# zhangyi-3/UCDIR

Hardware: AMD Instinct MI355X
Metric: restored images/sec at 50-step p_sample_loop, 256x256 SID (higher is better)
Workload: dtype bf16

## Files before the change

ucdir_amd/csrc/engine.hip:

```cpp
#include <hip/hip_runtime.h>

#include <cmath>
#include <cstdio>
#include <cstring>
#include <map>
#include <mutex>
#include <set>
#include <array>
#include <atomic>
#include <memory>
#include <string>
#include <vector>

#include "../../include/ucdir_hip.h"
#include "cgemm.hip.h"
#include "conv_halo.hip.h"
#include "akgm_halo.hip.h"
#include "akgm_pre.hip.h"
#include "akgm_ws.hip.h"
#include "akgm_ws32.hip.h"
#include "akgm_ws64.hip.h"
#include "conv_ws.hip.h"
#include "conv_sk.hip.h"
#include "conv_ws128.hip.h"
#include "flash_attn2.hip.h"
#include "qkv_ws.hip.h"
#include "common.h"
#include "misc.hip.h"
#include "fewstep.hip.h"
#include "image_metrics.hip.h"
#include "pack.h"

static thread_local std::string g_err;
static int fail(const std::string& m) { g_err = m; return 1; }
#define HIPC(x)                                                                                   \
    do {                                                                                          \
        hipError_t e_ = (x);                                                                      \
        if (e_ != hipSuccess) {                                                                   \
            throw std::runtime_error(std::string(#x) + ": " + hipGetErrorString(e_));             \
        }                                                                                         \
    } while (0)
#define API_BEGIN try {
#define API_END                                                                                   \
    }                                                                                             \
    catch (const std::exception& e) { return fail(e.what()); }                                    \
    catch (...) { return fail("unknown error"); }                                                 \
    return 0;

static void require(bool c, const std::string& m) { if (!c) throw std::runtime_error(m); }

struct DevGuard {
    int prev = -1; bool changed = false;
    explicit DevGuard(int dev) {
        HIPC(hipGetDevice(&prev));
        if (prev != dev) { HIPC(hipSetDevice(dev)); changed = true; }
    }
    ~DevGuard() { if (changed) (void)hipSetDevice(prev); }
};

struct DevPool {
    std::vector<void*> ptrs;
    int64_t bytes = 0;
    void* alloc(size_t n, bool zero = true) {
        void* p = nullptr;
        if (n == 0) n = 16;
        HIPC(hipMalloc(&p, n));
        if (zero) HIPC(hipMemset(p, 0, n));
        ptrs.push_back(p); bytes += (int64_t)n;
        return p;
    }
    template <typename T> T* upload(const std::vector<T>& v) {
        T* p = (T*)alloc(v.size() * sizeof(T), false);
        if (!v.empty()) HIPC(hipMemcpy(p, v.data(), v.size() * sizeof(T), hipMemcpyHostToDevice));
        return p;
    }
    static constexpr size_t STAT_CAP = 1 << 21;
    stat_t* stat_slab = nullptr; size_t stat_used = 0;
    stat_t* alloc_stats(int B) {
        if (!stat_slab) stat_slab = (stat_t*)alloc(STAT_CAP * sizeof(stat_t), true);
        const size_t n = (size_t)2 * UCDIR_STAT_SLOTS * B;
        if (stat_used + n > STAT_CAP) throw std::runtime_error("DevPool: statistics slab exhausted");
        stat_t* p = stat_slab + stat_used; stat_used += n;
        return p;
    }
    void zero_stats(hipStream_t st) { if (stat_used) HIPC(hipMemsetAsync(stat_slab, 0, stat_used * sizeof(stat_t), st)); }
    void release() { for (void* p : ptrs) (void)hipFree(p); ptrs.clear(); bytes = 0; stat_slab = nullptr; stat_used = 0; }
    ~DevPool() { release(); }
};

struct ConvW {
    bf16_t* A = nullptr; float* bias = nullptr; float* Tb = nullptr; float* Tg = nullptr;
    int rows_pad = 0, Kpad = 0, ntaps = 0, cin = 0, cout = 0, TM = 128; bool fold = false;
    bf16_t* Aup = nullptr; int Kup = 0;
    bf16_t* A10 = nullptr; float* bias_res = nullptr;
    bf16_t* Aws = nullptr;
    bf16_t* Aws128 = nullptr;
    bf16_t* Aqkv = nullptr;
    bf16_t* Atile = nullptr;
    bf16_t* Ask[2] = {nullptr, nullptr}; bf16_t* Ask_up[2] = {nullptr, nullptr};
    long long sk_up_stride[2] = {0, 0};
    bf16_t* Ask1x1 = nullptr;
};
struct AkgmW {
    bf16_t* A = nullptr; float* bias = nullptr; float* Tb = nullptr; float* Tg = nullptr;
    float* Tbb = nullptr;
    bf16_t* Apre = nullptr;
    bf16_t* Aws32 = nullptr;
    bf16_t* Aws64 = nullptr;
    int C = 0, cg = 0, Kpad = 0;
};

static int pick_tm(int cout) { return cout >= 128 ? 128 : 64; }

static ConvW upload_conv(DevPool& pool, const float* w, const float* bias, const float* gamma, const float* beta,
                         int cout, int cin, int ks) {
    ConvW W;
    W.TM = pick_tm(cout);
    PackedConv P = pack_conv(w, bias, gamma, beta, cout, cin, ks, W.TM);
    W.A = pool.upload(P.A); W.bias = pool.upload(P.bias);
    W.fold = gamma != nullptr;
    if (W.fold) { W.Tb = pool.upload(P.Tb); W.Tg = pool.upload(P.Tg); }
    W.rows_pad = P.rows_pad; W.Kpad = P.Kpad; W.ntaps = P.ntaps; W.cin = cin; W.cout = cout;
    if (ks == 3 && cin == 64 && cout == 64 && P.Kpad == 576) W.Aws = pool.upload(pack_conv_ws(P));
    if (ks == 3 && cin % 32 == 0 && P.Kpad == 9 * cin && P.rows_pad % W.TM == 0) W.Atile = pool.upload(pack_conv_tiled(P, W.TM));
    if (ks == 3 && cin % 32 == 0 && P.Kpad == 9 * cin && cout % 128 == 0) {
        W.Ask[0] = pool.upload(pack_conv_sk(P.A, 1, P.rows_pad, P.Kpad, cin, 9, 1));
        if (cout % 256 == 0) W.Ask[1] = pool.upload(pack_conv_sk(P.A, 1, P.rows_pad, P.Kpad, cin, 9, 2));
    }
    if (ks == 1 && cin % 32 == 0 && P.Kpad == cin && cout % 128 == 0 && gamma == nullptr) W.Ask1x1 = pool.upload(pack_conv_sk(P.A, 1, P.rows_pad, P.Kpad, cin, 1, 1));
    if (ks == 1 && cout == 3 * cin && gamma != nullptr && (cin == 256 || cin == 512) && P.Kpad == cin && P.rows_pad >= cout) W.Aqkv = pool.upload(pack_qkv_ws(P, cin));
    return W;
}
static void upload_upconv(DevPool& pool, ConvW& W, const float* w, const float* bias) {
    PackedConv P = pack_upconv(w, bias, W.cout, W.cin, W.TM);
    W.Aup = pool.upload(P.A); W.Kup = P.Kpad;
    for (int mw = 1; mw <= 2; ++mw)
        if (W.cin % 32 == 0 && W.cout % (128 * mw) == 0) {
            std::vector<bf16_t> img = pack_conv_sk(P.A, 4, P.rows_pad, P.Kpad, W.cin, 4, mw);
            W.sk_up_stride[mw - 1] = (long long)((img.size() - (size_t)4 * 4 * mw * 2 * 512) / 4);
            W.Ask_up[mw - 1] = pool.upload(img);
        }
}
static AkgmW upload_akgm(DevPool& pool, const float* wsp, const float* bsp, const float* gamma, const float* beta, int C) {
    PackedAkgm P = pack_akgm(wsp, bsp, gamma, beta, C, 0);
    AkgmW W;
    W.A = pool.upload(P.A); W.bias = pool.upload(P.bias); W.Tb = pool.upload(P.Tb); W.Tg = pool.upload(P.Tg);
    W.C = C; W.cg = P.cg; W.Kpad = P.Kpad;
    {
        std::vector<float> tbb(P.Tb.size());
// ... 11 lines not shown
struct Profiler {
    bool on = false;
    std::vector<ProfEntry> entries;
    std::vector<hipEvent_t> pool; size_t used = 0;
    hipEvent_t get() {
        if (used == pool.size()) { hipEvent_t e; HIPC(hipEventCreate(&e)); pool.push_back(e); }
        return pool[used++];
    }
    ~Profiler() { for (auto e : pool) (void)hipEventDestroy(e); }
};
static Profiler g_prof;

template <int TM, int EPI, int MODE>
static void launch_one(const GemmP& p, dim3 grid, size_t lds, hipStream_t st) {
    hipLaunchKernelGGL((cgemm_kernel<TM, EPI, MODE>), grid, dim3(CG_THREADS), lds, st, p);
}

template <typename K> static void set_lds_attr(K* k, int bytes, bool abs0 = false) {
    HIPC(hipFuncSetAttribute((const void*)k, hipFuncAttributeMaxDynamicSharedMemorySize, bytes));
    if (abs0) {
        hipFuncAttributes fa;
        HIPC(hipFuncGetAttributes(&fa, (const void*)k));
        require(fa.sharedSizeBytes == 0, "a kernel with absolute LDS addressing has static __shared__ memory: its dynamic smem[] no longer starts at offset 0");
    }
}
template <int TM> static void set_cgemm_attrs() {
    set_lds_attr(cgemm_kernel<TM, EPI_STD, MODE_S1>, 100 * 1024, true); set_lds_attr(cgemm_kernel<TM, EPI_STD, MODE_DOWN>, 100 * 1024, true);
    set_lds_attr(cgemm_kernel<TM, EPI_STD, MODE_UP>, 100 * 1024, true); set_lds_attr(cgemm_kernel<TM, EPI_STD, MODE_PLAIN>, 100 * 1024, true);
    set_lds_attr(cgemm_kernel<TM, EPI_STD, MODE_S1C>, 100 * 1024, true); set_lds_attr(cgemm_kernel<TM, EPI_AKGM, MODE_S1>, 100 * 1024, true);
}
#define SPLITK_MAX_WGS 512
#define SK_MAX_GRID 256
#define SCRATCH_BYTES ((size_t)2 * SK_MAX_GRID * 65536 * sizeof(float))
static std::map<int, float*> g_splitk_buf;
static std::mutex g_static_mu;
static void ensure_kernel_attrs() {
    std::lock_guard<std::mutex> lk(g_static_mu);
    static std::set<int> done;
    int dev = 0;
    HIPC(hipGetDevice(&dev));
    if (done.count(dev)) return;
    set_cgemm_attrs<64>(); set_cgemm_attrs<128>();
    set_lds_attr(conv3x3_halo_kernel<128, false>, hc_lds_bytes<128>());
    set_lds_attr(conv3x3_halo_kernel<64, false>, hc_lds_bytes<64>());
    set_lds_attr(conv3x3_halo_kernel<64, true>, hc_lds_bytes<64>());
    set_lds_attr(akgm_halo_stage_kernel, AH_LDS); set_lds_attr(akgm_halo_kernel<true>, AH_LDS);
    set_lds_attr(akgm_pre_kernel<8>, AkPre<8>::LDS);
    set_lds_attr(akgm_ws_kernel<8>, AkWs::LDS); set_lds_attr(akgm_ws_kernel<16>, AkWs::LDS);
    set_lds_attr(akgm_ws32_kernel<32>, AkWs32::LDS); set_lds_attr(akgm_ws32_kernel<16>, AkWs32::LDS); set_lds_attr(akgm_ws32_kernel<8>, AkWs32::LDS);
    set_lds_attr(akgm_ws64_kernel<2, 8, true>, 160 * 1024); set_lds_attr(akgm_ws64_kernel<4, 8, true>, 160 * 1024);
    set_lds_attr(qkv_ws_kernel<256>, QkvWs::LDS); set_lds_attr(qkv_ws_kernel<512>, QkvWs::LDS);
    set_lds_attr(conv_ws_kernel, CvWs::LDS);
    set_lds_attr(conv_ws128_kernel, CvWs128::LDS);
    set_lds_attr(conv_sk_kernel<2, 8, 9>, 160 * 1024); set_lds_attr(conv_sk_kernel<2, 8, 4>, 160 * 1024);
    set_lds_attr(conv_sk_kernel<1, 8, 9>, 160 * 1024); set_lds_attr(conv_sk_kernel<1, 8, 4>, 160 * 1024);
    set_lds_attr(conv_sk_kernel<1, 4, 9>, 80 * 1024, true); set_lds_attr(conv_sk_kernel<1, 4, 4>, 80 * 1024, true);

    set_lds_attr(final_conv_kernel, 160 * 1024);
    set_lds_attr(flash_attn2_kernel<1, false>, fa_lds_bytes(128), true); set_lds_attr(flash_attn2_kernel<1, true>, fa_lds_bytes(128), true);
    set_lds_attr(flash_attn2_kernel<2, false>, fa_lds_bytes(256), true); set_lds_attr(flash_attn2_kernel<2, true>, fa_lds_bytes(256), true);
    set_lds_attr(flash_attn2_kernel<3, false>, fa_lds_bytes(384), true); set_lds_attr(flash_attn2_kernel<3, true>, fa_lds_bytes(384), true);
    set_lds_attr(flash_attn2_kernel<4, false>, fa_lds_bytes(512), true); set_lds_attr(flash_attn2_kernel<4, true>, fa_lds_bytes(512), true);
    done.insert(dev);
}

static void gemm_work(const GemmP& p, int epi, double& flops, double& bytes) {
    const double cols = ((p.cols_mode == COLS_PLAIN) ? (double)p.W : (double)p.H * p.W) * (p.up_phase ? 4.0 : 1.0);
    if (epi == EPI_AKGM) {
        const double C = 8.0 * p.cg;
        flops = 2.0 * 9 * C * C * cols * p.nbatch;
        bytes = (2.0 * C * cols * 2 + C * cols * 2 + cols * 32) * p.nbatch + 9.0 * C * C * 2;
    } else {
        const double K = (double)p.ntaps * p.cg;
        flops = 2.0 * K * p.nfeat * cols * p.nbatch;
        double in_cols = cols;
        if (p.cols_mode == COLS_DOWN) in_cols = cols * 4; else if (p.cols_mode == COLS_UP) in_cols = cols / 4;
        bytes = ((double)p.cg * in_cols * 2 + (double)p.nfeat * cols * (p.out_f32 ? 4 : 2) + (p.res ? (double)p.nfeat * cols * 2 : 0)) * p.nbatch
                + (p.a_bstride ? (double)p.nfeat * K * 2 * p.nbatch : (double)p.nfeat * K * 2);
    }
}

static void launch_cgemm_impl(const GemmP& p, int TM, int epi, hipStream_t st);
static void launch_cgemm(const GemmP& p, int TM, int epi, hipStream_t st) {
    if (!g_prof.on) { launch_cgemm_impl(p, TM, epi, st); return; }
    ProfEntry e;
    int mode = p.cols_mode; if (mode == COLS_S1 && p.in_compact) mode = MODE_S1C;
    e.key = (TM == 128 ? 100 : 0) + (epi == EPI_AKGM ? 10 : 0) + (epi == EPI_AKGM ? 0 : mode);
    gemm_work(p, epi, e.flops, e.bytes);
    e.dH = p.H; e.dW = p.W; e.dCin = p.cg * p.ntaps; e.dCout = p.nfeat;
    e.e0 = g_prof.get(); e.e1 = g_prof.get();
    HIPC(hipEventRecord(e.e0, st));
    launch_cgemm_impl(p, TM, epi, st);
    HIPC(hipEventRecord(e.e1, st));
    g_prof.entries.push_back(e);
}

static void launch_cgemm_impl(const GemmP& p0, int TM, int epi, hipStream_t st) {
    GemmP p = p0;
#ifdef UCDIR_TIMING
    static unsigned long long* cgdbg = nullptr;
    if (!cgdbg) HIPC(hipMalloc((void**)&cgdbg, 64 * 8));
    HIPC(hipMemsetAsync(cgdbg, 0, 64 * 8, st));
    p.dbg = cgdbg;
    struct Pr { unsigned long long* d; hipStream_t s; int mode, TM, nk; ~Pr() {
        unsigned long long h[64]; (void)hipStreamSynchronize(s); (void)hipMemcpy(h, d, sizeof(h), hipMemcpyDeviceToHost);
        const int n = (int)h[63]; fprintf(stderr, "CGEMM TIMING mode=%d TM=%d nk=%d n=%d:", mode, TM, nk, n);
// ... 364 lines not shown
    if (!dbgbuf) HIPC(hipMalloc((void**)&dbgbuf, 256 * 8));
    HIPC(hipMemset(dbgbuf, 0, 256 * 8));
    p.dbg = dbgbuf;
#endif
    int tm_run = w.TM;
    if (halo && tm_run == 128 && p.nbatch * p.tiles * p.rowtiles < 256) {
        tm_run = 64; p.rowtiles = w.rows_pad / 64;
    }
    static const bool fuse_res = !getenv("UCDIR_NO_FUSED_RES");
    bool did_res = false;
    if (halo && !upph && tm_run == 64 && w.TM == 64 && w.A10 && res_out && fuse_res) {
        p.A = w.A10; p.a_ld = 10 * cin; p.res_fused = 1; p.bias2 = w.bias_res;
        p.out2 = res_out->p; p.out2_bstride = res_out->bstride(); p.out2_ld = res_out->C;
        did_res = true;
    }
    const bool dual = did_res;
    static const bool use_atile = !getenv("UCDIR_NO_ATILE");
    if (use_atile && halo && !upph && !did_res && tm_run == w.TM && w.Atile && w.ntaps == 9) p.A_tiled = w.Atile;
    static const bool use_cws128 = !getenv("UCDIR_NO_CONV_WS128");
    if (use_cws128 && did_res && w.Aws128 && cin == 128 && x0.C == 64 && x1 && x1->C == 64 && !res && !p.out_nchw && y.H % 8 == 0 && y.W % 16 == 0 &&
        y.C == 64 && (g_persist_grid > 0 || (long long)y.B * (y.H / 8) * (y.W / 16) >= 4LL * num_cus())) {
        p.A = w.Aws128; p.alt_A = w.Aws128 + (size_t)2 * 72 * 2 * 32 * 8;
        p.th = 8; p.tw = 16; p.tiles_x = y.W / 16; p.tiles_y = y.H / 8;
        const int ntiles = y.B * p.tiles_x * p.tiles_y, ncu = num_cus();
        const int grid = ntiles < ncu ? ntiles : ncu;
#ifdef UCDIR_TIMING
        {
            static unsigned long long* dbgbuf = nullptr;
            if (!dbgbuf) HIPC(hipMalloc((void**)&dbgbuf, 256 * 8));
            HIPC(hipMemset(dbgbuf, 0, 256 * 8));
            p.dbg = dbgbuf;
            hipLaunchKernelGGL(conv_ws128_kernel, dim3(grid), dim3(CvWs128::THREADS), CvWs128::LDS, st, p);
            unsigned long long h[256];
            HIPC(hipStreamSynchronize(st));
            HIPC(hipMemcpy(h, dbgbuf, sizeof(h), hipMemcpyDeviceToHost));
            const int n = (int)h[255];
            fprintf(stderr, "CONV_WS128 TIMING n=%d:", n);
            for (int i = 1; i < n && i < 255; ++i) fprintf(stderr, " %llu", h[i] - h[i - 1]);
            fprintf(stderr, "\n");
            return did_res;
        }
#endif
        if (g_prof.on) {
            ProfEntry e; e.key = 24; gemm_work(p, EPI_STD, e.flops, e.bytes);
            { const double cols = (double)p.H * p.W * p.nbatch; e.flops += 2.0 * p.cg * p.nfeat * cols; e.bytes += 2.0 * p.cg * p.nfeat + 2.0 * p.nfeat * cols; }
            e.dH = p.H; e.dW = p.W; e.dCin = p.cg; e.dCout = p.nfeat;
            e.e0 = g_prof.get(); e.e1 = g_prof.get();
            HIPC(hipEventRecord(e.e0, st));
            hipLaunchKernelGGL(conv_ws128_kernel, dim3(grid), dim3(CvWs128::THREADS), CvWs128::LDS, st, p);
            HIPC(hipEventRecord(e.e1, st));
            g_prof.entries.push_back(e);
        } else {
            hipLaunchKernelGGL(conv_ws128_kernel, dim3(grid), dim3(CvWs128::THREADS), CvWs128::LDS, st, p);
        }
        HIPC(hipGetLastError());
        return did_res;
    }
    if (halo && !did_res && !p.out_nchw && w.cout % 8 == 0) {
        const int taps = upph ? 4 : 9, tps = 256 / tm_run;
        const int ks = choose_ksplit(p.nbatch * p.tiles * p.rowtiles, cin / HC_BK, (taps + tps - 1) / tps,
                                     (double)y.B * y.H * y.W * w.cout);
        if (ks > 1) { p.ksplit = ks; p.partial = splitk_scratch(); }
    }
    static const bool tail_res = !getenv("UCDIR_NO_TAIL_RES");
    if (halo && !upph && !did_res && res_out && wres && tail_res && !p.out_nchw && wres->ntaps == 1 &&
        wres->rows_pad >= p.rowtiles * tm_run) {
        p.alt_blocks = p.nbatch * p.tiles * p.rowtiles;
        p.alt_A = wres->A; p.alt_a_ld = wres->Kpad; p.bias2 = wres->bias;
        p.out2 = res_out->p; p.out2_bstride = res_out->bstride(); p.out2_ld = res_out->C;
        did_res = true;
    }
    static const bool use_cws = !getenv("UCDIR_NO_CONV_WS");
    if (use_cws && halo && !upph && !did_res && !dual && w.Aws && !x1 && !res && !p.out_nchw && p.ksplit <= 1 && !p.alt_blocks &&
        y.H % 16 == 0 && y.W % 16 == 0 && x0.C == 64 && y.C == 64 &&
        (g_persist_grid > 0 || (long long)y.B * (y.H / 16) * (y.W / 16) >= 4LL * num_cus())) {
        p.A = w.Aws; p.th = 16; p.tw = 16; p.tiles_x = y.W / 16; p.tiles_y = y.H / 16;
        const int ntiles = y.B * p.tiles_x * p.tiles_y, ncu = num_cus();
        const int grid = ntiles < ncu ? ntiles : ncu;
#ifdef UCDIR_TIMING
        {
            static unsigned long long* dbgbuf = nullptr;
            if (!dbgbuf) HIPC(hipMalloc((void**)&dbgbuf, 512 * 8));
            HIPC(hipMemset(dbgbuf, 0, 512 * 8));
            p.dbg = dbgbuf;
            hipLaunchKernelGGL(conv_ws_kernel, dim3(grid), dim3(HC_THREADS), CvWs::LDS, st, p);
            unsigned long long h[512];
            HIPC(hipStreamSynchronize(st));
            HIPC(hipMemcpy(h, dbgbuf, sizeof(h), hipMemcpyDeviceToHost));
            for (int w = 0; w < 2; ++w) {
                const int n = (int)h[w * 256 + 255];
                fprintf(stderr, "CONV_WS TIMING %s n=%d:", w ? "late" : "early", n);
                for (int i = 1; i < n && i < 255; ++i) fprintf(stderr, " %llu", h[w * 256 + i] - h[w * 256 + i - 1]);
                fprintf(stderr, "\n");
            }
            return did_res;
        }
#endif
        if (g_prof.on) {
            ProfEntry e; e.key = 23; gemm_work(p, EPI_STD, e.flops, e.bytes);
            e.dH = p.H; e.dW = p.W; e.dCin = p.cg; e.dCout = p.nfeat;
            e.e0 = g_prof.get(); e.e1 = g_prof.get();
            HIPC(hipEventRecord(e.e0, st));
            hipLaunchKernelGGL(conv_ws_kernel, dim3(grid), dim3(HC_THREADS), CvWs::LDS, st, p);
            HIPC(hipEventRecord(e.e1, st));
            g_prof.entries.push_back(e);
        } else {
// ... 479 lines not shown
}

static const std::vector<float>& W_(ucdir_ctx* c, const std::string& name, size_t expect) {
    auto it = c->host.find(name);
    require(it != c->host.end(), "missing weight: " + name);
    require(it->second.v.size() == expect, "weight " + name + " has wrong size");
    return it->second.v;
}

static void finalize_weights(ucdir_ctx* c) {
    const auto& cfg = c->cfg;
    const int inner = cfg.inner_channel;
    c->wpool.release();
    c->lw.assign(c->layers.size(), LayerW());
    c->mlp_w1 = c->wpool.upload(W_(c, "noise_level_mlp.1.weight", (size_t)4 * inner * inner));
    c->mlp_b1 = c->wpool.upload(W_(c, "noise_level_mlp.1.bias", (size_t)4 * inner));
    c->mlp_w2 = c->wpool.upload(W_(c, "noise_level_mlp.3.weight", (size_t)4 * inner * inner));
    c->mlp_b2 = c->wpool.upload(W_(c, "noise_level_mlp.3.bias", (size_t)inner));
    std::vector<float> tw;
    int nb = 0;
    for (size_t li = 0; li < c->layers.size(); ++li) {
        const LayerDesc& d = c->layers[li];
        LayerW& w = c->lw[li];
        if (d.kind == "stem") {
            const auto& sw = W_(c, d.name + ".weight", (size_t)d.cout * d.cin * 9);
            require(d.cin == 6, "stem expects in_channel == 6 (cat[cond, x_t])");
            std::vector<float> t((size_t)54 * d.cout);
            for (int o = 0; o < d.cout; ++o) for (int ci = 0; ci < 6; ++ci) for (int k = 0; k < 9; ++k)
                t[(size_t)(k * 6 + ci) * d.cout + o] = sw[((size_t)o * 6 + ci) * 9 + k];
            require(d.cout % 64 == 0, "stem: inner_channel must be a multiple of 64");
            w.stem_w = c->wpool.upload(pack_stem_frags(t, W_(c, d.name + ".bias", (size_t)d.cout), 6, d.cout));
        } else if (d.kind == "down" || d.kind == "up") {
            w.conv = upload_conv(c->wpool, W_(c, d.name + ".conv.weight", (size_t)d.cout * d.cin * 9).data(),
                                 W_(c, d.name + ".conv.bias", d.cout).data(), nullptr, nullptr, d.cout, d.cin, 3);
            if (d.kind == "up") upload_upconv(c->wpool, w.conv, W_(c, d.name + ".conv.weight", (size_t)d.cout * d.cin * 9).data(),
                                              W_(c, d.name + ".conv.bias", d.cout).data());
        } else {
            const std::string r = d.name + ".res_block.";
            w.block_index = nb++;
            w.conv = upload_conv(c->wpool, W_(c, r + "conv1.weight", (size_t)d.cout * d.cin * 9).data(),
                                 W_(c, r + "conv1.bias", d.cout).data(), W_(c, r + "norm1.weight", d.cin).data(),
                                 W_(c, r + "norm1.bias", d.cin).data(), d.cout, d.cin, 3);
            w.has_res = d.cin != d.cout;
            if (w.has_res) {
                w.resconv = upload_conv(c->wpool, W_(c, r + "res_conv.weight", (size_t)d.cout * d.cin).data(),
                                        W_(c, r + "res_conv.bias", d.cout).data(), nullptr, nullptr, d.cout, d.cin, 1);
                if (w.conv.TM == 64 && d.cin % 64 == 0 && w.conv.Kpad == 9 * d.cin) {
                    PackedConv P = pack_conv(W_(c, r + "conv1.weight", (size_t)d.cout * d.cin * 9).data(), nullptr,
                                             W_(c, r + "norm1.weight", d.cin).data(), W_(c, r + "norm1.bias", d.cin).data(),
                                             d.cout, d.cin, 3, 64);
                    const std::vector<bf16_t> a10 = pack_conv_res10(P, W_(c, r + "res_conv.weight", (size_t)d.cout * d.cin).data());
                    w.conv.A10 = c->wpool.upload(a10);
                    if (d.cin == 128 && d.cout == 64) w.conv.Aws128 = c->wpool.upload(pack_conv_ws128(a10));
                    w.conv.bias_res = w.resconv.bias;
                }
            }
            w.sp = upload_akgm(c->wpool, W_(c, r + "spdyconv.weight", (size_t)8 * d.cout * (d.cout / 8) * 9).data(),
                               W_(c, r + "spdyconv.bias", (size_t)8 * d.cout).data(), W_(c, r + "norm2.weight", d.cout).data(),
                               W_(c, r + "norm2.bias", d.cout).data(), d.cout);
            std::vector<float> gw;
            for (const char* s : {"conv2.0.weight", "conv2.0.bias", "conv2.2.weight", "conv2.2.bias"}) {
                const auto& v = c->host.at(r + s).v;
                gw.insert(gw.end(), v.begin(), v.end());
            }
            require(gw.size() == 48 + 16 + 576 + 8, "guide branch weights have wrong size");
            w.gw = c->wpool.upload(gw);
            for (const char* s : {"noise_func.0.weight", "noise_func.0.bias", "noise_func.2.weight", "noise_func.2.bias"}) {
                const auto& v = c->host.at(r + s).v;
                tw.insert(tw.end(), v.begin(), v.end());
            }
            if (d.attn) {
                const std::string a = d.name + ".attn.";
                const std::vector<float> wf = fold_out_into_v(W_(c, a + "qkv.weight", (size_t)3 * d.cout * d.cout).data(),
                                                              W_(c, a + "out.weight", (size_t)d.cout * d.cout).data(), d.cout);
                w.qkv = upload_conv(c->wpool, wf.data(), nullptr,
                                    W_(c, a + "norm.weight", d.cout).data(), W_(c, a + "norm.bias", d.cout).data(),
                                    3 * d.cout, d.cout, 1);
                w.outp = upload_conv(c->wpool, W_(c, a + "out.weight", (size_t)d.cout * d.cout).data(),
                                     W_(c, a + "out.bias", d.cout).data(), nullptr, nullptr, d.cout, d.cout, 1);
            }
        }
    }
    c->nblocks = nb;
    require(tw.size() == (size_t)nb * (8 * inner + 8 + 64 + 8), "time weights have wrong size");
    c->tw = c->wpool.upload(tw);
    const int fc = inner * cfg.channel_mults[0];
    c->fin_gamma = c->wpool.upload(W_(c, "final_conv.0.weight", fc));
    c->fin_beta = c->wpool.upload(W_(c, "final_conv.0.bias", fc));
    c->fin_conv = upload_conv(c->wpool, W_(c, "final_conv.3.weight", (size_t)cfg.out_channel * fc * 9).data(),
                              W_(c, "final_conv.3.bias", cfg.out_channel).data(), nullptr, nullptr, cfg.out_channel, fc, 3);
    if (cfg.out_channel <= 4 && fc % 32 == 0) {
        c->fin_w = c->wpool.upload(pack_final_frags(W_(c, "final_conv.3.weight", (size_t)cfg.out_channel * fc * 9).data(), cfg.out_channel, fc));
        c->fin_b = c->wpool.upload(W_(c, "final_conv.3.bias", cfg.out_channel));
    }
    c->host.clear();
    c->finalized = true;
}

static int level_dim(int d, int level) { return d >> level; }

struct ActPlanner {
    DevPool& pool; int B; bool reuse;
    std::map<std::array<int, 3>, std::vector<bf16_t*>> free_;
    Act get(int h, int w, int C, bool stats = true) {
        Act a; a.B = B; a.H = h; a.W = w; a.C = C;
        auto& fl = free_[{h, w, C}];
// ... 581 lines not shown
}

int32_t ucdir_op_conv(const float* x0, int32_t c0, const float* x1, int32_t c1, int32_t B, int32_t H, int32_t W,
                      const float* w_host, const float* bias_host, const float* gamma_host, const float* beta_host,
                      int32_t cout, int32_t ksize, int32_t mode, int32_t silu, const float* residual, float* y,
                      double* stats_out_host, void* stream) {
    API_BEGIN
    ensure_kernel_attrs();
    hipStream_t st = (hipStream_t)stream;
    DevPool pool;
    Act a0 = act_from_nchw(pool, x0, B, c0, H, W, st, true);
    Act a1; if (x1) a1 = act_from_nchw(pool, x1, B, c1, H, W, st, true);
    int Ho = H, Wo = W;
    if (mode == COLS_DOWN) { Ho = H / 2; Wo = W / 2; } else if (mode == COLS_UP) { Ho = 2 * H; Wo = 2 * W; }
    Act out = make_act(pool, B, Ho, Wo, cout);
    Act res; if (residual) res = act_from_nchw(pool, residual, B, cout, Ho, Wo, st, false);
    ConvW w = upload_conv(pool, w_host, bias_host, gamma_host, beta_host, cout, c0 + (x1 ? c1 : 0), ksize);
    if (mode == COLS_UP && ksize == 3) upload_upconv(pool, w, w_host, bias_host);
    run_conv(w, a0, x1 ? &a1 : nullptr, out, mode, silu, residual ? &res : nullptr, true, st);
    hipLaunchKernelGGL(act_to_nchw_kernel, dim3(2048), dim3(256), 0, st, out.p, y, B, cout, Ho, Wo);
    HIPC(hipGetLastError());
    std::vector<stat_t> sfx;
    if (stats_out_host) { sfx.resize((size_t)2 * UCDIR_STAT_SLOTS * B); HIPC(hipMemcpyAsync(sfx.data(), out.stats, sizeof(stat_t) * sfx.size(), hipMemcpyDeviceToHost, st)); }
    HIPC(hipStreamSynchronize(st));
    if (stats_out_host)
        for (int bb = 0; bb < B; ++bb)
            for (int q = 0; q < 2; ++q) {
                stat_t acc = 0;
                for (int k = 0; k < UCDIR_STAT_SLOTS; ++k) acc += sfx[((size_t)bb * UCDIR_STAT_SLOTS + k) * 2 + q];
                stats_out_host[bb * 2 + q] = (double)acc / UCDIR_STAT_SCALE;
            }
    API_END
}

int32_t ucdir_op_conv_res(const float* x0, int32_t c0, const float* x1, int32_t c1, int32_t B, int32_t H, int32_t W,
                          const float* w_host, const float* bias_host, const float* gamma_host, const float* beta_host,
                          const float* wres_host, const float* bres_host, int32_t cout, int32_t silu,
                          float* y, float* yres, double* stats_out_host, void* stream) {
    API_BEGIN
    ensure_kernel_attrs();
    hipStream_t st = (hipStream_t)stream;
    DevPool pool;
    const int cin = c0 + (x1 ? c1 : 0);
    Act a0 = act_from_nchw(pool, x0, B, c0, H, W, st, true);
    Act a1; if (x1) a1 = act_from_nchw(pool, x1, B, c1, H, W, st, true);
    Act out = make_act(pool, B, H, W, cout), rout = make_act(pool, B, H, W, cout, false);
    ConvW w = upload_conv(pool, w_host, bias_host, gamma_host, beta_host, cout, cin, 3);
    ConvW wr = upload_conv(pool, wres_host, bres_host, nullptr, nullptr, cout, cin, 1);
    if (w.TM == 64 && cin % 64 == 0 && w.Kpad == 9 * cin) {
        PackedConv P = pack_conv(w_host, nullptr, gamma_host, beta_host, cout, cin, 3, 64);
        const std::vector<bf16_t> a10 = pack_conv_res10(P, wres_host);
        w.A10 = pool.upload(a10); w.bias_res = wr.bias;
        if (cin == 128 && cout == 64) w.Aws128 = pool.upload(pack_conv_ws128(a10));
    }
    const bool did = run_conv(w, a0, x1 ? &a1 : nullptr, out, COLS_S1, silu, nullptr, true, st, nullptr, 0, 0, &rout, &wr);
    if (!did) run_conv(wr, a0, x1 ? &a1 : nullptr, rout, COLS_S1, 0, nullptr, false, st);
    hipLaunchKernelGGL(act_to_nchw_kernel, dim3(2048), dim3(256), 0, st, out.p, y, B, cout, H, W);
    hipLaunchKernelGGL(act_to_nchw_kernel, dim3(2048), dim3(256), 0, st, rout.p, yres, B, cout, H, W);
    HIPC(hipGetLastError());
    std::vector<stat_t> sfx;
    if (stats_out_host) { sfx.resize((size_t)2 * UCDIR_STAT_SLOTS * B); HIPC(hipMemcpyAsync(sfx.data(), out.stats, sizeof(stat_t) * sfx.size(), hipMemcpyDeviceToHost, st)); }
    HIPC(hipStreamSynchronize(st));
    if (stats_out_host)
        for (int bb = 0; bb < B; ++bb)
            for (int q = 0; q < 2; ++q) {
                stat_t acc = 0;
                for (int k = 0; k < UCDIR_STAT_SLOTS; ++k) acc += sfx[((size_t)bb * UCDIR_STAT_SLOTS + k) * 2 + q];
                stats_out_host[bb * 2 + q] = (double)acc / UCDIR_STAT_SCALE;
            }
    API_END
}

int32_t ucdir_op_akgm(const float* h, const float* att, const float* res, int32_t B, int32_t C, int32_t H, int32_t W,
                      const float* wsp_host, const float* bsp_host, const float* gamma_host, const float* beta_host,
                      float* y, double* stats_out_host, void* stream) {
    API_BEGIN
    ensure_kernel_attrs();
    hipStream_t st = (hipStream_t)stream;
    DevPool pool;
    Act ah = act_from_nchw(pool, h, B, C, H, W, st, true);
    Act ar = act_from_nchw(pool, res, B, C, H, W, st, false);
    Act out = make_act(pool, B, H, W, C);
    float* G = (float*)pool.alloc((size_t)B * H * W * 8 * 4);
    hipLaunchKernelGGL(nchw8_to_compact_kernel, dim3(1024), dim3(256), 0, st, att, G, B, H, W);
    std::vector<float> ones((size_t)B * 8, 1.f);
    float* attw = pool.upload(ones);
    AkgmW w = upload_akgm(pool, wsp_host, bsp_host, gamma_host, beta_host, C);
    float* tcbuf = (float*)pool.alloc((size_t)B * (9 * 8 * C + 2) * sizeof(float), false);
    run_akgm(w, ah, G, attw, ar, out, tcbuf, st);
    hipLaunchKernelGGL(act_to_nchw_kernel, dim3(2048), dim3(256), 0, st, out.p, y, B, C, H, W);
    HIPC(hipGetLastError());
    std::vector<stat_t> sfx;
    if (stats_out_host) { sfx.resize((size_t)2 * UCDIR_STAT_SLOTS * B); HIPC(hipMemcpyAsync(sfx.data(), out.stats, sizeof(stat_t) * sfx.size(), hipMemcpyDeviceToHost, st)); }
    HIPC(hipStreamSynchronize(st));
    if (stats_out_host)
        for (int bb = 0; bb < B; ++bb)
            for (int q = 0; q < 2; ++q) {
                stat_t acc = 0;
                for (int k = 0; k < UCDIR_STAT_SLOTS; ++k) acc += sfx[((size_t)bb * UCDIR_STAT_SLOTS + k) * 2 + q];
                stats_out_host[bb * 2 + q] = (double)acc / UCDIR_STAT_SCALE;
            }
    API_END
}

int32_t ucdir_op_attention(const float* x, int32_t B, int32_t C, int32_t H, int32_t W, const float* gamma_host,
                           const float* beta_host, const float* wqkv_host, const float* wout_host, const float* bout_host,
// ... 265 lines not shown
```

ucdir_amd/csrc/pack.h:

```cpp
#pragma once
#include <cmath>
#include <cstdint>
#include <vector>

#include "common.h"

struct PackedConv {
    std::vector<bf16_t> A;
    std::vector<float> bias;
    std::vector<float> Tb, Tg;
    int rows_pad = 0, Kpad = 0, ntaps = 0, cin = 0, cout = 0, ncls = 0;
};

static inline bool tap_valid(int cls, int tap) {
    const int cy = cls / 3, cx = cls % 3, ky = tap / 3, kx = tap % 3;
    if (cy == 0 && ky == 0) return false;
    if (cy == 2 && ky == 2) return false;
    if (cx == 0 && kx == 0) return false;
    if (cx == 2 && kx == 2) return false;
    return true;
}

static inline PackedConv pack_conv(const float* w, const float* bias, const float* gamma, const float* beta,
                                   int cout, int cin, int ks, int TM) {
// ... 14 lines not shown
                const float ws = fold ? wv * gamma[c] : wv;
                const bf16_t q = f2bf(ws);
                P.A[(size_t)o * P.Kpad + (size_t)t * cin + c] = q;
                if (fold) {
                    wb[(size_t)t * cout + o] += (double)wv * beta[c];
                    wg[(size_t)t * cout + o] += (double)bf2f(q);
                }
            }
    if (fold) {
        P.Tb.assign((size_t)P.ncls * cout, 0.f);
        P.Tg.assign((size_t)P.ncls * cout, 0.f);
        for (int cls = 0; cls < P.ncls; ++cls)
            for (int o = 0; o < cout; ++o) {
                double sb = 0, sg = 0;
                for (int t = 0; t < P.ntaps; ++t) {
                    const int t9 = (P.ntaps == 9) ? t : 4;
                    if (P.ncls == 9 && !tap_valid(cls, t9)) continue;
                    sb += wb[(size_t)t * cout + o]; sg += wg[(size_t)t * cout + o];
                }
                P.Tb[(size_t)cls * cout + o] = (float)sb;
                P.Tg[(size_t)cls * cout + o] = (float)sg;
            }
    }
    return P;
}

static inline std::vector<bf16_t> pack_conv_ws(const PackedConv& P) {
    std::vector<bf16_t> img((size_t)2 * 36 * 2 * 32 * 8, 0);
    for (int rw = 0; rw < 2; ++rw)
        for (int j = 0; j < 36; ++j)
            for (int hk = 0; hk < 2; ++hk)
                for (int rho = 0; rho < 32; ++rho) {
                    const int o = 32 * rw + 16 * ((rho >> 2) & 1) + (rho & 3) + 4 * (rho >> 3);
                    const int tap = j >> 2, c0 = 16 * (j & 3) + 8 * hk;
                    for (int e = 0; e < 8; ++e)
                        img[((((size_t)rw * 36 + j) * 2 + hk) * 32 + rho) * 8 + e] = P.A[(size_t)o * P.Kpad + (size_t)tap * 64 + c0 + e];
                }
    return img;
}

static inline std::vector<bf16_t> pack_conv_ws128(const std::vector<bf16_t>& A10) {
    const int K10 = 10 * 128, nj = 80;
    std::vector<bf16_t> img((size_t)2 * nj * 2 * 32 * 8, 0);
    for (int rw = 0; rw < 2; ++rw)
        for (int j = 0; j < nj; ++j)
            for (int hk = 0; hk < 2; ++hk)
                for (int rho = 0; rho < 32; ++rho) {
                    const int o = 32 * rw + 16 * ((rho >> 2) & 1) + (rho & 3) + 4 * (rho >> 3);
                    const int tap = j >> 3, c0 = 16 * (j & 7) + 8 * hk;
                    const size_t dst = j < 72 ? ((((size_t)rw * 72 + j) * 2 + hk) * 32 + rho) * 8
                                              : (size_t)2 * 72 * 2 * 32 * 8 + ((((size_t)rw * 8 + (j - 72)) * 2 + hk) * 32 + rho) * 8;
                    for (int e = 0; e < 8; ++e) img[dst + e] = A10[(size_t)o * K10 + (size_t)tap * 128 + c0 + e];
                }
    return img;
}

static inline std::vector<bf16_t> pack_conv_res10(const PackedConv& P, const float* wres) {
    const int cin = P.cin, K10 = 10 * cin;
    std::vector<bf16_t> A((size_t)P.rows_pad * K10, 0);
    for (int o = 0; o < P.rows_pad; ++o) {
        for (int k = 0; k < 9 * cin; ++k) A[(size_t)o * K10 + k] = P.A[(size_t)o * P.Kpad + k];
        if (o < P.cout)
            for (int c = 0; c < cin; ++c) A[(size_t)o * K10 + 9 * cin + c] = f2bf(wres[(size_t)o * cin + c]);
    }
    return A;
}

struct PackedAkgm {
    std::vector<bf16_t> A;
    std::vector<float> bias;
    std::vector<float> Tb, Tg;
    int C = 0, cg = 0, Kpad = 0;
};

static inline PackedAkgm pack_akgm(const float* wsp, const float* bsp, const float* gamma, const float* beta, int C,
                                   int kpad_override = 0) {
    PackedAkgm P;
    P.C = C; P.cg = C / 8;
    const int cg = P.cg;
    const bool chunked = (cg == 64) && !kpad_override;
    P.Kpad = kpad_override ? kpad_override : (chunked ? 640 : ((9 * cg + 63) / 64) * 64);
    P.A.assign((size_t)8 * C * P.Kpad, 0);
    P.bias.assign((size_t)8 * C, 0.f);
    P.Tb.assign((size_t)9 * 8 * C, 0.f);
    P.Tg.assign((size_t)9 * 8 * C, 0.f);
    for (int o = 0; o < 8 * C; ++o) P.bias[o] = bsp[o];
    for (int g = 0; g < 8; ++g)
        for (int pr = 0; pr < C; ++pr) {
            const int t32 = pr / 32, rho = pr % 32;
            const int floc = 4 * t32 + ((rho >> 4) & 1) * 2 + ((rho >> 2) & 1);
            const int s = (rho & 3) + 4 * ((rho >> 3) & 1);
            const int o = g * C + 8 * floc + s;
            bf16_t* row = &P.A[((size_t)g * C + pr) * P.Kpad];
            double wb[9] = {0}, wg[9] = {0};
            for (int ci = 0; ci < cg; ++ci) {
                const int cglob = g * cg + ci;
                for (int t = 0; t < 9; ++t) {
                    const float wv = wsp[((size_t)o * cg + ci) * 9 + t];
                    const bf16_t q = f2bf(wv * gamma[cglob]);
                    row[chunked ? (size_t)(ci / 32) * 320 + (size_t)t * 32 + (ci % 32) : (size_t)t * cg + ci] = q;
                    wb[t] += (double)wv * beta[cglob];
                    wg[t] += (double)bf2f(q);
                }
            }
            for (int cls = 0; cls < 9; ++cls) {
                double sb = 0, sg = 0;
// ... 178 lines not shown
```

Baseline: 37.16.

## Add persistent weight-stationary fused conv+residual kernel for 192->64 channel blocks

Adds a persistent, weight-stationary 3x3 conv kernel for cin=192 (128+64 concatenated inputs) to cout=64 with a fused 1x1 residual conv. It keeps the packed weights in registers, double-buffers input halos in LDS via async DMA, and splits K across 4 wave groups with an LDS cross-wave reduction. The epilogue applies the group-norm fold, activation and stats accumulation. It targets the decoder concat blocks that previously went through the generic halo/split-K path, at the cost of heavy register and LDS pressure and more barriers.

```diff
diff --git a/ucdir_amd/csrc/conv_wsk.hip.h b/ucdir_amd/csrc/conv_wsk.hip.h
--- /dev/null
+++ b/ucdir_amd/csrc/conv_wsk.hip.h
@@ -0,0 +1,297 @@
+#pragma once
+#include <type_traits>
+#include "conv_ws.hip.h"
+
+struct CvWsk {
+    static constexpr int PITCH = 24;
+    static constexpr int PLANE = 6 * PITCH * 128;
+    static constexpr int HALO = 3 * PLANE;
+    static constexpr int QSTEP = 2 * PITCH * 128;
+    static constexpr int NSTEP = 30;
+    static constexpr int SLOT = 4096;
+    static constexpr int SLOTS_IN_BUF = HALO / SLOT;
+    static constexpr int OFF_RX = 2 * HALO;
+    static constexpr int OFF_TCS = OFF_RX + (24 - SLOTS_IN_BUF) * SLOT;
+    static constexpr int OFF_B2 = OFF_TCS + 9 * 64 * 4;
+    static constexpr int OFF_SCAL = OFF_B2 + 64 * 4;
+    static constexpr int LDS = OFF_SCAL + 128;
+    static constexpr int THREADS = 512;
+    static constexpr int DEPTH = 2;
+    static constexpr int A_ELEMS = 2 * 4 * NSTEP * 2 * 32 * 8;
+};
+static_assert(CvWsk::LDS <= 160 * 1024, "conv_wsk: LDS budget");
+static_assert(CvWsk::OFF_RX + (24 - CvWsk::SLOTS_IN_BUF) * CvWsk::SLOT <= CvWsk::OFF_TCS, "conv_wsk: partial slots");
+
+__global__ __launch_bounds__(CvWsk::THREADS, 2) void conv_wsk_kernel(const GemmP p) {
+    using L = CvWsk;
+    extern __shared__ __attribute__((aligned(16))) unsigned char smem[];
+    float* const tcs = reinterpret_cast<float*>(smem + L::OFF_TCS);
+    float* const b2s = reinterpret_cast<float*>(smem + L::OFF_B2);
+    float* const scal = reinterpret_cast<float*>(smem + L::OFF_SCAL);
+    const int tid = threadIdx.x, lane = tid & 63, l31 = lane & 31, hh = lane >> 5;
+    const int wave = __builtin_amdgcn_readfirstlane(tid >> 6);
+    const int rw = wave & 1, kq = wave >> 1;
+    const int prow = l31 >> 4, pcol = (l31 & 15) ^ (prow << 3);
+    int lid;
+    {
+        const int nblk = gridDim.x, bid = blockIdx.x;
+        const int q = nblk >> 3, r = nblk & 7, xcd = bid & 7;
+        lid = (xcd < r ? xcd * (q + 1) : r * (q + 1) + (xcd - r) * q) + (bid >> 3);
+    }
+#ifdef UCDIR_TIMING
+    const bool dbg_on = p.dbg && (lid == (int)gridDim.x / 2 + 3) && (lane == 0) && (wave == 1);
+    int dbg_n = 0;
+#define CK_STAMP() do { if (dbg_on && dbg_n < 250) p.dbg[dbg_n++] = __builtin_amdgcn_s_memtime(); } while (0)
+#else
+#define CK_STAMP() do {} while (0)
+#endif
+    CK_STAMP();
+    const int tps = p.tiles_x * p.tiles_y;
+    const int T = p.nbatch * tps;
+    const int t_beg = (int)((long long)lid * T / (int)gridDim.x), t_end = (int)((long long)(lid + 1) * T / (int)gridDim.x);
+    if (t_beg >= t_end) return;
+
+    bf16x8_t af[L::NSTEP];
+    {
+        const bf16_t* Ab = p.A + (((rw * 4 + kq) * L::NSTEP * 2 + hh) * 32 + l31) * 8;
+#pragma unroll
+        for (int j = 0; j < L::NSTEP; ++j) af[j] = *reinterpret_cast<const bf16x8_t*>(Ab + j * (2 * 32 * 8));
+    }
+#pragma unroll
+    for (int j = 0; j < L::NSTEP; ++j) asm volatile("" : "+v"(af[j]));
+    if (tid < 64) b2s[tid] = p.bias2 ? p.bias2[tid] : 0.f;
+
+    const int lcol = lane >> 3, lch = lane & 7;
+    auto piece = [&](auto plc, int k, const unsigned char* base, unsigned hoff) __attribute__((always_inline)) {
+        constexpr int pl = decltype(plc)::value;
+        const int q = 8 * k + wave;
+        if (q < 18) {
+            const int r = q / 3, c3 = q - 3 * r;
+            const int col = min(8 * c3 + lcol, 17), hp = r * L::PITCH + col;
+            const unsigned voff = ((unsigned)(r * p.Wp + col) << (pl < 2 ? 8 : 7))
+                                + ((unsigned)(lch ^ ((hp >> 1) & 7)) << 4);
+            dma16_sbase(base, voff, (unsigned)__builtin_amdgcn_readfirstlane(hoff + pl * L::PLANE + (3 * r + c3) * 1024));
+        }
+    };
+    auto plane_base = [&](int nb, int nty, int ntx, int pl) __attribute__((always_inline)) -> const unsigned char* {
+        const long long pix0 = (long long)nty * 4 * p.Wp + ntx * 16;
+        if (pl < 2) return reinterpret_cast<const unsigned char*>(p.B0 + (long long)nb * p.b0_bstride + pix0 * 128 + pl * 64);
+        return reinterpret_cast<const unsigned char*>(p.B1 + (long long)nb * p.b1_bstride + pix0 * 64);
+    };
+    unsigned ba[3], bb[3];
+    {
+        const int hp0 = prow * L::PITCH + pcol;
+#pragma unroll
+        for (int kx = 0; kx < 3; ++kx) {
+            const int sxh = (((hp0 + kx) >> 1) & 7) ^ hh;
+            ba[kx] = ((hp0 + kx) << 7) + (((2 * kq) ^ sxh) << 4);
+            bb[kx] = ((hp0 + kx) << 7) + (((2 * (kq ^ 2)) ^ sxh) << 4);
+        }
+    }
+    const bool own_res = kq >= 2;
+    const unsigned tc_lane = L::OFF_TCS + (32 * rw + 16 * hh) * 4;
+    const unsigned b2_lane = L::OFF_B2 + (32 * rw + 16 * hh) * 4;
+
+    int b, ty, tx;
+    {
+        b = t_beg / tps;
+        const int r = t_beg - b * tps;
+        ty = r / p.tiles_x; tx = r - ty * p.tiles_x;
+    }
+    static_for<0, 3>([&](auto plc) __attribute__((always_inline)) {
+        const unsigned char* const base = plane_base(b, ty, tx, decltype(plc)::value);
+        for (int k = 0; k < 3; ++k) piece(plc, k, base, 0u);
+    });
+
+    int b_cur = -1;
+    float rstd_a = 1.f;
+    stat_t S1 = 0, S2 = 0;
+    const int act = p.act;
+
+#pragma unroll 1
+    for (int t = t_beg; t < t_end; ++t) {
+        const int buf = (t - t_beg) & 1;
+        const bool last = t + 1 == t_end;
+        CK_STAMP();
+        if (t == t_beg) { HC_WAIT(0); }
+        asm volatile("s_barrier" ::: "memory");
+        CK_STAMP();
+        if (b != b_cur) {
+            if (b_cur >= 0 && p.stats_out && !own_res) {
+                const stat_t a = wave_sum_ll(S1), q2 = wave_sum_ll(S2);
+                if (lane == 0) stat_add_fx(p.stats_out, b_cur, a, q2);
+            }
+            S1 = 0; S2 = 0;
+            b_cur = b;
+            if (wave == 0) {
+                float mean = 0.f, rstd = 1.f;
+                if (p.fold) {
+                    long long v = 0;
+                    if (lane < 2 * UCDIR_STAT_SLOTS) {
+                        v = p.stats0[(long long)b * (2 * UCDIR_STAT_SLOTS) + lane];
+                        if (p.stats1) v += p.stats1[(long long)b * (2 * UCDIR_STAT_SLOTS) + lane];
+                    }
+#pragma unroll
+                    for (int off = 2; off < 2 * UCDIR_STAT_SLOTS; off <<= 1) v += __shfl_xor(v, off);
+                    const long long q = __shfl(v, 1);
+                    mean_rstd(stat_val(v), stat_val(q), p.inv_count, mean, rstd);
+                }
+                if (lane == 0) { scal[0] = mean; scal[1] = rstd; }
+            }
+            __syncthreads();
+            const float mean = scal[0], rstd = scal[1];
+            for (int i = tid; i < 9 * 64; i += L::THREADS) {
+                const int cls = i >> 6, f = i & 63;
+                float v = p.bias ? p.bias[f] : 0.f;
+                if (p.fold) v += p.Tb[(long long)cls * p.tab_ld + f] - mean * rstd * p.Tg[(long long)cls * p.tab_ld + f];
+                tcs[i] = v;
+            }
+            rstd_a = __builtin_bit_cast(float, __builtin_amdgcn_readfirstlane(__builtin_bit_cast(int, p.alpha * (p.fold ? rstd : 1.0f))));
+            __syncthreads();
+        }
+        int nb = b, nty = ty, ntx = tx + 1;
+        if (ntx == p.tiles_x) { ntx = 0; if (++nty == p.tiles_y) { nty = 0; ++nb; } }
+        CK_STAMP();
+
+        if (t != t_beg) {
+            const int d = buf ? L::HALO : -L::HALO;
+#pragma unroll
+            for (int kx = 0; kx < 3; ++kx) { ba[kx] += d; bb[kx] += d; }
+        }
+
+        f32x16_t acc[2], acc2[2];
+        {
+            bf16x8_t bq[L::DEPTH + 1][2];
+            const unsigned char* const nbase0 = plane_base(nb, nty, ntx, 0);
+            const unsigned char* const nbase1 = plane_base(nb, nty, ntx, 1);
+            const unsigned char* const nbase2 = plane_base(nb, nty, ntx, 2);
+            const unsigned hd = (unsigned)((buf ^ 1) * L::HALO);
+            __builtin_amdgcn_sched_barrier(0);
+            asm volatile("s_waitcnt lgkmcnt(0)" ::: "memory");
+            auto read_b = [&](auto jc, bf16x8_t (&dst)[2]) __attribute__((always_inline)) {
+                constexpr int j = decltype(jc)::value;
+                constexpr int pl = j < 27 ? j / 9 : j - 27, tap = j < 27 ? j % 9 : 4, ky = tap / 3, kx = tap - 3 * ky;
+                constexpr int off = pl * L::PLANE + ky * (L::PITCH * 128);
+                const unsigned a = ky == 1 ? bb[kx] : ba[kx];
+                lds_read16_asm<off>(dst[0], a);
+                lds_read16_asm<off + L::QSTEP>(dst[1], a);
+            };
+            static_for<0, L::DEPTH>([&](auto jc) __attribute__((always_inline)) { read_b(jc, bq[decltype(jc)::value]); });
+            static_for<0, L::NSTEP>([&](auto jc) __attribute__((always_inline)) {
+                constexpr int j = decltype(jc)::value;
+                if constexpr (j + L::DEPTH < L::NSTEP) read_b(std::integral_constant<int, j + L::DEPTH>{}, bq[(j + L::DEPTH) % (L::DEPTH + 1)]);
+                if constexpr (j % 3 == 1 && j / 3 < 9) {
+                    constexpr int i = j / 3, pl = i / 3;
+                    if (!last) piece(std::integral_constant<int, pl>{}, i % 3, pl == 0 ? nbase0 : (pl == 1 ? nbase1 : nbase2), hd);
+                }
+                constexpr int ahead = (L::NSTEP - 1 - j) < L::DEPTH ? (L::NSTEP - 1 - j) : L::DEPTH;
+                lgkm_wait_asm<2 * ahead>();
+                const f32x16_t zero = {0.f, 0.f, 0.f, 0.f, 0.f, 0.f, 0.f, 0.f, 0.f, 0.f, 0.f, 0.f, 0.f, 0.f, 0.f, 0.f};
+                const bf16x8_t(&bv)[2] = bq[j % (L::DEPTH + 1)];
+                if constexpr (j < 27) {
+                    acc[0] = __builtin_amdgcn_mfma_f32_32x32x16_bf16(af[j], bv[0], j ? acc[0] : zero, 0, 0, 0);
+                    acc[1] = __builtin_amdgcn_mfma_f32_32x32x16_bf16(af[j], bv[1], j ? acc[1] : zero, 0, 0, 0);
+                } else {
+                    acc2[0] = __builtin_amdgcn_mfma_f32_32x32x16_bf16(af[j], bv[0], j > 27 ? acc2[0] : zero, 0, 0, 0);
+                    acc2[1] = __builtin_amdgcn_mfma_f32_32x32x16_bf16(af[j], bv[1], j > 27 ? acc2[1] : zero, 0, 0, 0);
+                }
+            });
+            __builtin_amdgcn_sched_barrier(0);
+        }
+        CK_STAMP();
+        asm volatile("s_barrier" ::: "memory");
+        CK_STAMP();
+
+        const unsigned slot_lane = lane * 16;
+        auto slot_addr = [&](int s) __attribute__((always_inline)) -> unsigned {
+            return (s < L::SLOTS_IN_BUF ? (unsigned)(buf * L::HALO + s * L::SLOT) : (unsigned)(L::OFF_RX + (s - L::SLOTS_IN_BUF) * L::SLOT)) + slot_lane;
+        };
+        auto put = [&](int u, const f32x16_t& v) __attribute__((always_inline)) {
+            const unsigned a = slot_addr(3 * (4 * rw + u) + (kq < u ? kq : kq - 1));
+#pragma unroll
+            for (int g4 = 0; g4 < 4; ++g4)
+                *reinterpret_cast<f32x4_t*>(smem + a + 1024 * g4) = f32x4_t{v[4 * g4], v[4 * g4 + 1], v[4 * g4 + 2], v[4 * g4 + 3]};
+        };
+        auto finish = [&](auto uc) __attribute__((always_inline)) {
+            constexpr int u = decltype(uc)::value, tp = u & 1;
+            constexpr bool is_res = u >= 2;
+            if constexpr (u != 0) put(0, acc[0]);
+            if constexpr (u != 1) put(1, acc[1]);
+            if constexpr (u != 2) put(2, acc2[0]);
+            if constexpr (u != 3) put(3, acc2[1]);
+            f32x16_t v = is_res ? acc2[tp] : acc[tp];
+            asm volatile("s_waitcnt lgkmcnt(0)\n\ts_barrier" ::: "memory");
+            CK_STAMP();
+#pragma unroll
+            for (int i = 0; i < 3; ++i) {
+                const unsigned a = slot_addr(3 * (4 * rw + u) + i);
+#pragma unroll
+                for (int g4 = 0; g4 < 4; ++g4) {
+                    const f32x4_t c4 = *reinterpret_cast<const f32x4_t*>(smem + a + 1024 * g4);
+#pragma unroll
+                    for (int e = 0; e < 4; ++e) v[4 * g4 + e] += c4[e];
+                }
+            }
+
+            const long long tile_el = (long long)(ty * 4 * p.Wp + tx * 16) * 64;
+            const unsigned rel_out = (unsigned)(((2 * tp + prow + 1) * p.Wp + pcol + 1) * 64 + 32 * rw + 16 * hh) * 2;
+            uint4 pk[2];
+            unsigned char* ob;
+            float o[16];
+            if constexpr (!is_res) {
+                const bool interior = ty > 0 && tx > 0 && ty + 1 < p.tiles_y && tx + 1 < p.tiles_x;
+                unsigned tca = tc_lane + 4 * 256;
+                if (!interior) {
+                    const int r = 2 * tp + prow, c = pcol;
+                    const int cy = (ty == 0 && r == 0) ? 0 : ((ty + 1 == p.tiles_y && r == 3) ? 2 : 1);
+                    const int cx = (tx == 0 && c == 0) ? 0 : ((tx + 1 == p.tiles_x && c == 15) ? 2 : 1);
+                    tca = tc_lane + (cy * 3 + cx) * 256;
+                }
+#pragma unroll
+                for (int g4 = 0; g4 < 4; ++g4) {
+                    const f32x4_t c4 = *reinterpret_cast<const f32x4_t*>(smem + tca + 16 * g4);
+#pragma unroll
+                    for (int e = 0; e < 4; ++e) o[4 * g4 + e] = fmaf(v[4 * g4 + e], rstd_a, c4[e]);
+                }
+                if (act == 1) {
+#pragma unroll
+                    for (int i = 0; i < 16; ++i) o[i] = silu_fast(o[i]);
+                } else if (act == 2) {
+#pragma unroll
+                    for (int i = 0; i < 16; ++i) o[i] = fmaxf(0.2f * o[i], o[i]);
+                }
+                float s1 = 0.f, s2 = 0.f;
+#pragma unroll
+                for (int i = 0; i < 16; ++i) { s1 += o[i]; s2 += o[i] * o[i]; }
+                S1 += stat_fx((double)s1); S2 += stat_fx((double)s2);
+                ob = reinterpret_cast<unsigned char*>(reinterpret_cast<bf16_t*>(p.out) + (long long)b * p.out_bstride + tile_el);
+            } else {
+#pragma unroll
+                for (int g4 = 0; g4 < 4; ++g4) {
+                    const f32x4_t d4 = *reinterpret_cast<const f32x4_t*>(smem + b2_lane + 16 * g4);
+#pragma unroll
+                    for (int e = 0; e < 4; ++e) o[4 * g4 + e] = v[4 * g4 + e] + d4[e];
+                }
+                ob = reinterpret_cast<unsigned char*>(p.out2 + (long long)b * p.out2_bstride + tile_el);
+            }
+            pk[0] = pack8_bf16(o); pk[1] = pack8_bf16(o + 8);
+            CK_STAMP();
+            HC_WAIT(0);
+            CK_STAMP();
+            *reinterpret_cast<uint4*>(ob + rel_out) = pk[0];
+            *reinterpret_cast<uint4*>(ob + rel_out + 16) = pk[1];
+        };
+        if (kq == 0) finish(std::integral_constant<int, 0>{});
+        else if (kq == 1) finish(std::integral_constant<int, 1>{});
+        else if (kq == 2) finish(std::integral_constant<int, 2>{});
+        else finish(std::integral_constant<int, 3>{});
+        b = nb; ty = nty; tx = ntx;
+    }
+#ifdef UCDIR_TIMING
+    if (dbg_on) p.dbg[255] = dbg_n;
+#endif
+    if (p.stats_out && !own_res) {
+        const stat_t a = wave_sum_ll(S1), q2 = wave_sum_ll(S2);
+        if (lane == 0) stat_add_fx(p.stats_out, b_cur, a, q2);
+    }
+}
diff --git a/ucdir_amd/csrc/engine.hip b/ucdir_amd/csrc/engine.hip
--- a/ucdir_amd/csrc/engine.hip
+++ b/ucdir_amd/csrc/engine.hip
@@ -23,6 +23,7 @@
 #include "conv_ws.hip.h"
 #include "conv_sk.hip.h"
 #include "conv_ws128.hip.h"
+#include "conv_wsk.hip.h"
 #include "flash_attn2.hip.h"
 #include "qkv_ws.hip.h"
 #include "common.h"
@@ -95,6 +96,7 @@
     bf16_t* A10 = nullptr; float* bias_res = nullptr;
     bf16_t* Aws = nullptr;
     bf16_t* Aws128 = nullptr;
+    bf16_t* Awsk = nullptr;
     bf16_t* Aqkv = nullptr;
     bf16_t* Atile = nullptr;
     bf16_t* Ask[2] = {nullptr, nullptr}; bf16_t* Ask_up[2] = {nullptr, nullptr};
@@ -212,6 +214,7 @@
     set_lds_attr(qkv_ws_kernel<256>, QkvWs::LDS); set_lds_attr(qkv_ws_kernel<512>, QkvWs::LDS);
     set_lds_attr(conv_ws_kernel, CvWs::LDS);
     set_lds_attr(conv_ws128_kernel, CvWs128::LDS);
+    set_lds_attr(conv_wsk_kernel, CvWsk::LDS);
     set_lds_attr(conv_sk_kernel<2, 8, 9>, 160 * 1024); set_lds_attr(conv_sk_kernel<2, 8, 4>, 160 * 1024);
     set_lds_attr(conv_sk_kernel<1, 8, 9>, 160 * 1024); set_lds_attr(conv_sk_kernel<1, 8, 4>, 160 * 1024);
     set_lds_attr(conv_sk_kernel<1, 4, 9>, 80 * 1024, true); set_lds_attr(conv_sk_kernel<1, 4, 4>, 80 * 1024, true);
@@ -682,6 +685,44 @@
             g_prof.entries.push_back(e);
         } else {
             hipLaunchKernelGGL(conv_ws128_kernel, dim3(grid), dim3(CvWs128::THREADS), CvWs128::LDS, st, p);
+        }
+        HIPC(hipGetLastError());
+        return did_res;
+    }
+    if (use_cws128 && did_res && w.Awsk && cin == 192 && x0.C == 128 && x1 && x1->C == 64 && !res && !p.out_nchw && y.H % 4 == 0 &&
+        y.W % 16 == 0 && y.C == 64 && (g_persist_grid > 0 || (long long)y.B * (y.H / 4) * (y.W / 16) >= 4LL * num_cus())) {
+        p.A = w.Awsk;
+        p.th = 4; p.tw = 16; p.tiles_x = y.W / 16; p.tiles_y = y.H / 4;
+        const int ntiles = y.B * p.tiles_x * p.tiles_y, ncu = num_cus();
+        const int grid = ntiles < ncu ? ntiles : ncu;
+#ifdef UCDIR_TIMING
+        {
+            static unsigned long long* dbgbuf = nullptr;
+            if (!dbgbuf) HIPC(hipMalloc((void**)&dbgbuf, 256 * 8));
+            HIPC(hipMemset(dbgbuf, 0, 256 * 8));
+            p.dbg = dbgbuf;
+            hipLaunchKernelGGL(conv_wsk_kernel, dim3(grid), dim3(CvWsk::THREADS), CvWsk::LDS, st, p);
+            unsigned long long h[256];
+            HIPC(hipStreamSynchronize(st));
+            HIPC(hipMemcpy(h, dbgbuf, sizeof(h), hipMemcpyDeviceToHost));
+            const int n = (int)h[255];
+            fprintf(stderr, "CONV_WSK TIMING n=%d:", n);
+            for (int i = 1; i < n && i < 255; ++i) fprintf(stderr, " %llu", h[i] - h[i - 1]);
+            fprintf(stderr, "\n");
+            return did_res;
+        }
+#endif
+        if (g_prof.on) {
+            ProfEntry e; e.key = 25; gemm_work(p, EPI_STD, e.flops, e.bytes);
+            { const double cols = (double)p.H * p.W * p.nbatch; e.flops += 2.0 * p.cg * p.nfeat * cols; e.bytes += 2.0 * p.cg * p.nfeat + 2.0 * p.nfeat * cols; }
+            e.dH = p.H; e.dW = p.W; e.dCin = p.cg; e.dCout = p.nfeat;
+            e.e0 = g_prof.get(); e.e1 = g_prof.get();
+            HIPC(hipEventRecord(e.e0, st));
+            hipLaunchKernelGGL(conv_wsk_kernel, dim3(grid), dim3(CvWsk::THREADS), CvWsk::LDS, st, p);
+            HIPC(hipEventRecord(e.e1, st));
+            g_prof.entries.push_back(e);
+        } else {
+            hipLaunchKernelGGL(conv_wsk_kernel, dim3(grid), dim3(CvWsk::THREADS), CvWsk::LDS, st, p);
         }
         HIPC(hipGetLastError());
         return did_res;
@@ -1267,6 +1308,7 @@
                     const std::vector<bf16_t> a10 = pack_conv_res10(P, W_(c, r + "res_conv.weight", (size_t)d.cout * d.cin).data());
                     w.conv.A10 = c->wpool.upload(a10);
                     if (d.cin == 128 && d.cout == 64) w.conv.Aws128 = c->wpool.upload(pack_conv_ws128(a10));
+                    if (d.cin == 192 && d.cout == 64) w.conv.Awsk = c->wpool.upload(pack_conv_wsk(a10));
                     w.conv.bias_res = w.resconv.bias;
                 }
             }
@@ -1954,6 +1996,7 @@
         const std::vector<bf16_t> a10 = pack_conv_res10(P, wres_host);
         w.A10 = pool.upload(a10); w.bias_res = wr.bias;
         if (cin == 128 && cout == 64) w.Aws128 = pool.upload(pack_conv_ws128(a10));
+        if (cin == 192 && cout == 64) w.Awsk = pool.upload(pack_conv_wsk(a10));
     }
     const bool did = run_conv(w, a0, x1 ? &a1 : nullptr, out, COLS_S1, silu, nullptr, true, st, nullptr, 0, 0, &rout, &wr);
     if (!did) run_conv(wr, a0, x1 ? &a1 : nullptr, rout, COLS_S1, 0, nullptr, false, st);
diff --git a/ucdir_amd/csrc/pack.h b/ucdir_amd/csrc/pack.h
--- a/ucdir_amd/csrc/pack.h
+++ b/ucdir_amd/csrc/pack.h
@@ -90,6 +90,22 @@
                                               : (size_t)2 * 72 * 2 * 32 * 8 + ((((size_t)rw * 8 + (j - 72)) * 2 + hk) * 32 + rho) * 8;
                     for (int e = 0; e < 8; ++e) img[dst + e] = A10[(size_t)o * K10 + (size_t)tap * 128 + c0 + e];
                 }
+    return img;
+}
+
+static inline std::vector<bf16_t> pack_conv_wsk(const std::vector<bf16_t>& A10) {
+    const int K10 = 10 * 192, ns = 30;
+    std::vector<bf16_t> img((size_t)2 * 4 * ns * 2 * 32 * 8, 0);
+    for (int rw = 0; rw < 2; ++rw)
+        for (int kq = 0; kq < 4; ++kq)
+            for (int s = 0; s < ns; ++s)
+                for (int hk = 0; hk < 2; ++hk)
+                    for (int rho = 0; rho < 32; ++rho) {
+                        const int o = 32 * rw + 16 * ((rho >> 2) & 1) + (rho & 3) + 4 * (rho >> 3);
+                        const int pl = s < 27 ? s / 9 : s - 27, tap = s < 27 ? s % 9 : 9, c0 = 64 * pl + 16 * kq + 8 * hk;
+                        const size_t dst = (((((size_t)rw * 4 + kq) * ns + s) * 2 + hk) * 32 + rho) * 8;
+                        for (int e = 0; e < 8; ++e) img[dst + e] = A10[(size_t)o * K10 + (size_t)tap * 192 + c0 + e];
+                    }
     return img;
 }
 
```

Result: no change. 37.27, median of 6 (+0.3%).
